# Yawning/secp256k1-voi

Measured on NVIDIA B200. Metric: ecdsa_verifies_per_sec, higher is better.
Workload: dtype u32 limbs (8x32, IMAD.WIDE.U32 carry chains)

## Files before the change

### secp256k1-voi_b200/csrc/api.cu

```cuda
#include "ctx.h"
#include "microbench.cuh"

__global__ void __launch_bounds__(S256_TPB) k_gen_table(apt *out, int wb, size_t total) {
    size_t idx = (size_t)blockIdx.x * blockDim.x + threadIdx.x;
    if (idx >= total) return;
    uint32_t w = (uint32_t)(idx >> wb), d = (uint32_t)(idx & ((1u << wb) - 1u));
    apt a;
    item_gen_multiple(a, w, d, wb);
    out[idx] = a;
}
__global__ void k_comb_bases(apt *bases) {
    uint32_t w = threadIdx.x;
    if (w < (uint32_t)COMB_NW) item_gen_multiple(bases[w], w, 1u, COMB_WB);
}
constexpr int COMB_RUN = 32;
static_assert(COMB_SZ % COMB_RUN == 0, "a run never straddles two windows");
__global__ void __launch_bounds__(S256_TPB) k_gen_comb(const apt *bases, size_t total, apt *out) {
    size_t e0 = ((size_t)blockIdx.x * blockDim.x + threadIdx.x) * COMB_RUN;
    if (e0 >= total) return;
    const apt B = bases[e0 / COMB_SZ];
    const uint32_t m = (uint32_t)(e0 % COMB_SZ) + 1u;
    pt buf[COMB_RUN];
    pt acc;
    pt_set_identity(acc);
// ... 16 lines not shown
    }
    fe_invert(inv, run);
#pragma unroll 1
    for (int i = COMB_RUN - 1; i >= 0; i--) {
        fe zi;
        apt a;
        fe_mul(zi, inv, pre[i]);
        fe_mul(inv, inv, buf[i].z);
        fe_mul(a.x, buf[i].x, zi);
        fe_mul(a.y, buf[i].y, zi);
        fe_normalize(a.x, a.x);
        fe_normalize(a.y, a.y);
        out[e0 + i] = a;
    }
}
template <int WB>
__global__ void __launch_bounds__(S256_TPB) k_gen_ct_table(apt *out) {
    constexpr int CT_SZ = ct_cfg<WB>::SZ, CT_NW = ct_cfg<WB>::NW, CT_WB = WB;
    uint32_t idx = blockIdx.x * blockDim.x + threadIdx.x;
    if (idx >= (uint32_t)(CT_NW * CT_SZ)) return;
    apt a;
    item_gen_multiple(a, idx / CT_SZ, idx % CT_SZ + 1u, CT_WB);
    out[idx] = a;
}

__global__ void __launch_bounds__(S256_TPB) k_decode_uncompressed(const uint8_t *pt65, size_t n, apt *aff,
                                                                  uint8_t *pvalid) {
    size_t i = (size_t)blockIdx.x * blockDim.x + threadIdx.x;
    if (i >= n) return;
    apt a;
    pvalid[i] = item_decode_uncompressed(a, pt65 + 65 * i);
    aff[i] = a;
}

__global__ void __launch_bounds__(S256_TPB) k_decode_compressed(const uint8_t *pt33, size_t n, apt *aff,
                                                                uint8_t *pvalid) {
    size_t i = (size_t)blockIdx.x * blockDim.x + threadIdx.x;
    if (i >= n) return;
    apt a;
    pvalid[i] = item_decode_compressed(a, pt33 + 33 * i);
    aff[i] = a;
}
__global__ void __launch_bounds__(S256_TPB) k_decode_sec1(const uint8_t *enc65, const uint8_t *len, size_t n, apt *aff,
                                                          uint8_t *pvalid) {
    size_t i = (size_t)blockIdx.x * blockDim.x + threadIdx.x;
    if (i >= n) return;
    const uint8_t *e = enc65 + 65 * i;
    apt a;
    a.x = fe_zero();
    a.y = fe_zero();
    uint8_t st = ST_INVALID;
    if (len[i] == 65)
        st = item_decode_uncompressed(a, e) ? ST_OK : ST_INVALID;
    else if (len[i] == 33)
        st = item_decode_compressed(a, e) ? ST_OK : ST_INVALID;
    else if (len[i] == 1 && e[0] == 0x00)
        st = ST_IDENTITY;
    pvalid[i] = st;
    aff[i] = a;
}
__global__ void __launch_bounds__(S256_TPB) k_encode_affine(const apt *aff, const uint8_t *pvalid, size_t n,
                                                            uint8_t *out65, uint8_t *status) {
    size_t i = (size_t)blockIdx.x * blockDim.x + threadIdx.x;
    if (i >= n) return;
    apt a = aff[i];
    uint32_t ok = pvalid[i] != 0;
    uint8_t *o = out65 + 65 * i;
    if (ok) {
        o[0] = 0x04;
        fe_to_be32(o + 1, a.x);
        fe_to_be32(o + 33, a.y);
    } else {
        for (int b = 0; b < 65; b++) o[b] = 0;
    }
    status[i] = ok ? ST_OK : ST_INVALID;
}
__global__ void __launch_bounds__(S256_TPB) k_encode_compressed(const apt *aff, const uint8_t *pvalid, size_t n,
                                                                uint8_t *out33, uint8_t *status) {
    size_t i = (size_t)blockIdx.x * blockDim.x + threadIdx.x;
    if (i >= n) return;
    apt a = aff[i];
    uint32_t ok = pvalid[i] != 0;
    uint8_t *o = out33 + 33 * i;
    if (ok) {
        o[0] = (uint8_t)(0x02u | fe_is_odd(a.y));
        fe_to_be32(o + 1, a.x);
    } else {
        for (int b = 0; b < 33; b++) o[b] = 0;
    }
    status[i] = ok ? ST_OK : ST_INVALID;
}
__global__ void __launch_bounds__(S256_TPB) k_encode_public_key(const apt *aff, const uint8_t *pvalid, size_t n,
                                                                uint8_t *out65, uint8_t *status) {
    size_t i = (size_t)blockIdx.x * blockDim.x + threadIdx.x;
    if (i >= n) return;
    apt a = aff[i];
    uint8_t *o = out65 + 65 * i;
    if (pvalid[i] == ST_OK) {
        o[0] = 0x04;
        fe_to_be32(o + 1, a.x);
        fe_to_be32(o + 33, a.y);
    } else {
        for (int b = 0; b < 65; b++) o[b] = 0;
    }
    status[i] = pvalid[i];
}

__global__ void __launch_bounds__(S256_TPB) k_decode_xonly(const uint8_t *pkx32, size_t n, apt *aff, uint8_t *pvalid) {
    size_t i = (size_t)blockIdx.x * blockDim.x + threadIdx.x;
    if (i >= n) return;
    apt a;
    pvalid[i] = item_decode_xonly(a, pkx32 + 32 * i);
    aff[i] = a;
}

__global__ void __launch_bounds__(S256_TPB) k_decode_recover(const uint8_t *sig65, size_t n, apt *aff,
                                                             uint8_t *pvalid) {
    size_t i = (size_t)blockIdx.x * blockDim.x + threadIdx.x;
    if (i >= n) return;
    apt a;
    pvalid[i] = item_decode_recover(a, sig65 + 65 * i);
    aff[i] = a;
}

template <int K, bool RECOVER>
__global__ void __launch_bounds__(S256_TPB, 4) k_ecdsa_scalars(const uint8_t *digest32, const uint8_t *sig, size_t n,
                                                            uint32_t flags, sc *u1, int8_t *dig1, int8_t *dig2,
                                                            uint8_t *sfl) {
    size_t stride = (n + K - 1) / K;
    size_t t = (size_t)blockIdx.x * blockDim.x + threadIdx.x;
    if (t >= stride) return;
    if (!RECOVER)
        group_ecdsa_scalars<K>(t, stride, n, digest32, sig, flags, u1, dig1, dig2, sfl);
    else
        group_recover_scalars<K>(t, stride, n, digest32, sig, u1, dig1, dig2, sfl);
}

__global__ void __launch_bounds__(S256_TPB) k_plain_scalars(const uint8_t *u1b, const uint8_t *u2b, size_t n, sc *u1,
                                                            int8_t *dig1, int8_t *dig2, uint8_t *sfl) {
    size_t i = (size_t)blockIdx.x * blockDim.x + threadIdx.x;
    if (i >= n) return;
    item_plain_scalars(i, n, u1b, u2b, u1, dig1, dig2, sfl);
}

__global__ void __launch_bounds__(S256_TPB) k_schnorr_scalars(const uint8_t *pkx32, const uint8_t *msg, size_t msg_len,
                                                              const uint8_t *sig64, size_t n, sc *u1, int8_t *dig1,
                                                              int8_t *dig2, uint8_t *sfl) {
    size_t i = (size_t)blockIdx.x * blockDim.x + threadIdx.x;
    if (i >= n) return;
    item_schnorr_scalars(i, n, pkx32, msg, msg_len, sig64, u1, dig1, dig2, sfl);
}

#ifndef S256_DSM_MINB
#define S256_DSM_MINB 4
#endif
#ifndef S256_DSM_TPB
#define S256_DSM_TPB S256_TPB
#endif
__device__ __forceinline__ void fe_shfl_xor(fe &r, const fe &a, int m) {
#pragma unroll
    for (int k = 0; k < 8; k++) r.v[k] = __shfl_xor_sync(0xFFFFFFFFu, a.v[k], m);
}
template <int TPB, class F>
__device__ __forceinline__ void cta_invert(F &f, fe &inv, const fe &c, fe *sh) {
    constexpr int PER = TPB / 32;
    sh[threadIdx.x] = c;
    __syncthreads();
    if (threadIdx.x < 32) {
        fe *mine = sh + threadIdx.x * PER;
        fe pre[PER];
        pre[0] = mine[0];
#pragma unroll
        for (int k = 1; k < PER; k++) f.mul(pre[k], pre[k - 1], mine[k]);
        fe all = pre[PER - 1], others, got;
        fe_shfl_xor(others, all, 1);
        f.mul(all, all, others);
#pragma unroll 1
        for (int m = 2; m < 32; m <<= 1) {
            fe_shfl_xor(got, all, m);
            f.mul(others, others, got);
            f.mul(all, all, got);
        }
        fe o;
        fe_invert(o, all);
        f.mul(o, o, others);
#pragma unroll
        for (int k = PER - 1; k >= 1; k--) {
            fe ck = mine[k], t;
            f.mul(t, o, pre[k - 1]);
            f.mul(o, o, ck);
            mine[k] = t;
        }
        mine[0] = o;
    }
    __syncthreads();
    inv = sh[threadIdx.x];
}
__global__ void __launch_bounds__(S256_DSM_TPB, S256_DSM_MINB)
    k_dsm(size_t n, const apt *aff, const sc *u1, const int8_t *dig1, const int8_t *dig2, const uint8_t *sfl, pt *tbl,
          pt *res, const apt *comb) {
    size_t i = (size_t)blockIdx.x * blockDim.x + threadIdx.x;
    if (i >= n) return;
    item_dsm(i, n, aff, u1, dig1, dig2, sfl, tbl, res, comb);
}

#ifndef S256_SM_MINB
#define S256_SM_MINB 4
#endif
__global__ void __launch_bounds__(S256_TPB, S256_SM_MINB)
    k_scalar_mult_ct(size_t n, const apt *aff, const uint8_t *k32, pt *tbl, pt *res) {
    size_t i = (size_t)blockIdx.x * blockDim.x + threadIdx.x;
#ifdef S256_CT_TABLE_GLOBAL
    if (i >= n) return;
    CtTableGlobal T{tbl + i * (size_t)DSM_TSTRIDE};
    item_scalar_mult_ct_affine(i, aff, k32, T, tbl + i * (size_t)DSM_TSTRIDE, res);
#else
    extern __shared__ uint4 ct_smem[];
    fe *sh = reinterpret_cast<fe *>(ct_smem);
    const bool live = i < n;
    fe_ops<true> f;
    fe zprod = fe_one(), inv;
    if (live) item_ctm_table(i, aff, tbl + i * (size_t)DSM_TSTRIDE, zprod);
    cta_invert<S256_TPB>(f, inv, zprod, sh);
    __syncthreads();
    if (!live) return;
    CtTableShared<S256_TPB> T{threadIdx.x, aff + i};
    item_ctm_ladder(i, aff, k32, T, tbl + i * (size_t)DSM_TSTRIDE, inv, res);
#endif
}
#ifdef S256_CT_TABLE_GLOBAL
constexpr size_t CT_SMEM_BYTES = 0;
#else
constexpr size_t CT_SMEM_BYTES = (size_t)(CTM_TS - 1) * 4 * S256_TPB * sizeof(uint4);
#endif
void s256_launch_scalar_mult_ct(size_t n, const apt *aff, const uint8_t *k32, pt *tbl, pt *res, cudaStream_t s) {
    if (n == 0) return;
    k_scalar_mult_ct<<<(unsigned)((n + S256_TPB - 1) / S256_TPB), S256_TPB, CT_SMEM_BYTES, s>>>(n, aff, k32, tbl, res);
}


__global__ void __launch_bounds__(S256_TPB) k_ecdsa_finish(size_t n, const pt *res, const uint8_t *sig64,
                                                           const uint8_t *pvalid, const uint8_t *sfl, uint8_t *ok) {
    size_t i = (size_t)blockIdx.x * blockDim.x + threadIdx.x;
    if (i >= n) return;
    pt R = res[i];
    uint32_t valid = (uint32_t)(pvalid[i] != 0) & (uint32_t)(sfl[i] & SFL_VALID);
    ok[i] = item_ecdsa_finish(R, sig64 + 64 * i, valid);
}

template <int K>
__global__ void __launch_bounds__(S256_TPB) k_finish_affine(size_t n, const pt *res, const uint8_t *pvalid,
                                                            const uint8_t *sfl, uint8_t *comb_status, int mode,
                                                            uint8_t *out, uint8_t *status, const uint8_t *sig64) {
    __shared__ uint4 stage[S256_TPB / 32][130];
    size_t stride = (((n + K - 1) / K) + 31) & ~(size_t)31;
    size_t t = (size_t)blockIdx.x * blockDim.x + threadIdx.x;
    if (t >= stride) return;
    group_finish<K>(t, stride, n, res, pvalid, sfl, comb_status, mode, out, status, sig64,
                    reinterpret_cast<uint8_t *>(stage[threadIdx.x / 32]));
}

__global__ void __launch_bounds__(S256_TPB) k_field_op(int op, const uint8_t *a32, const uint8_t *b32, size_t n,
                                                       uint8_t *out32) {
    size_t i = (size_t)blockIdx.x * blockDim.x + threadIdx.x;
    if (i >= n) return;
    if (op < 16 || op >= 20) {
        fe a, b, r;
        fe_from_be32(a, a32 + 32 * i);
        fe_from_be32(b, b32 + 32 * i);
        switch (op) {
            case 0: fe_mul(r, a, b); break;
            case 1: fe_add(r, a, b); break;
            case 2: fe_sub(r, a, b); break;
            case 3: fe_invert(r, a); break;
            case 4: fe_sqrt(r, a); break;
            case 5: fe_mul_small(r, a, 21u); break;
            case 6: fe_sqr(r, a); break;
            case 7: fe_invert_fermat(r, a); break;
            case 8: fe_mul_vt(r, a, b); break;
            case 9: fe_add_vt(r, a, b); break;
            case 10: fe_sub_vt(r, a, b); break;
            case 13: fe_mul_small_vt(r, a, 21u); break;
            case 14: fe_sqr_vt(r, a); break;
            case 15: fe_mul8_vt(r, a); break;
            case 20: fe_mul2_vt(r, a); break;
            case 21: fe_mul3_vt(r, a); break;
            case 22: fe_sub2_vt(r, a, b); break;
            case 23: fe_submul8_vt(r, a, b); break;
            case 24: fe_ops<false>::mul2add(r, a, b, b, a); break;
            case 25: fe_ops<false>::mul2sub(r, a, a, b, b); break;
            default: r = fe_zero();
        }
        fe_normalize(r, r);
        fe_to_be32(out32 + 32 * i, r);
    } else {
        sc a, b, r;
        sc_from_be32(a, a32 + 32 * i);
        sc_from_be32(b, b32 + 32 * i);
        switch (op) {
            case 16: sc_mul(r, a, b); break;
            case 17: sc_add(r, a, b); break;
            case 18: sc_invert(r, a); break;
            case 19: sc_invert_fermat(r, a); break;
            default: r = sc_zero();
        }
        sc_to_be32(out32 + 32 * i, r);
    }
}

extern "C" void *s256_host_alloc(size_t bytes) {
    void *p = nullptr;
    if (cudaHostAlloc(&p, bytes ? bytes : 1, cudaHostAllocPortable) != cudaSuccess) {
        cudaGetLastError();
        return nullptr;
    }
    return p;
}
extern "C" void s256_host_free(void *p) {
    if (p) cudaFreeHost(p);
}

extern "C" const char *s256_strerror(int code) {
    switch (code) {
        case S256_SUCCESS: return "success";
        case S256_ERR_NO_DEVICE: return "no usable CUDA device (sm_100 required; there is no CPU fallback)";
        case S256_ERR_CUDA: return "CUDA runtime error";
        case S256_ERR_ARG: return "invalid argument";
        case S256_ERR_NOMEM: return "out of memory";
        case S256_ERR_UNIMPLEMENTED: return "not implemented";
        case S256_ERR_NCCL: return "NCCL error";
        default: return "unknown error";
    }
}
extern "C" const char *s256_last_cuda_error(const s256_ctx *ctx) { return ctx ? ctx->last_err.c_str() : ""; }
extern "C" int s256_device(const s256_ctx *ctx) { return ctx ? ctx->device : -1; }
extern "C" uint64_t s256_launch_count(const s256_ctx *ctx) { return ctx ? ctx->launches.load() : 0; }

extern "C" void s256_free(s256_ctx *ctx) {
    if (!ctx) return;
    {
        dev_guard g(ctx->device);
        s256_internal_comm_release(ctx);
        void *ptrs[] = {ctx->comb, ctx->ct_tab, ctx->ct_tab_small, ctx->ct_tab_huge, ctx->aff, ctx->u1,   ctx->dig1, ctx->dig2, ctx->sfl, ctx->pvalid,
                        ctx->cstat, ctx->tbl,   ctx->res, ctx->in_a, ctx->in_b, ctx->in_c, ctx->out, ctx->st,
                        ctx->sink, ctx->msm_counts, ctx->msm_offsets, ctx->msm_cursor, ctx->msm_entries, ctx->msm_flag,
                        ctx->msm_buckets, ctx->msm_win, ctx->msm_acc, ctx->msm_tmp, ctx->msm_cub, ctx->msm_nsl, ctx->msm_sloff,
                        ctx->msm_perm, ctx->msm_hist, ctx->msm_range, ctx->msm_part, ctx->msm_sbkt, ctx->comm_buf, ctx->msm_aff2, ctx->msm_half, ctx->msm_bsum};
        for (void *p : ptrs)
            if (p) cudaFree(p);
        if (ctx->stream) cudaStreamDestroy(ctx->stream);
        if (ctx->stream2) cudaStreamDestroy(ctx->stream2);
        if (ctx->ev_decode) cudaEventDestroy(ctx->ev_decode);
        if (ctx->ev_idle) cudaEventDestroy(ctx->ev_idle);
        for (cudaEvent_t e : ctx->ev_pipe)
// ... 880 lines not shown
```

### secp256k1-voi_b200/csrc/jac.cuh

```cuda
#pragma once
#include "point.cuh"

namespace s256 {

template <class F>
S256_HD void jac_double(F &fo, pt &v, const pt &p) {
    fe a, b, c, d, e, f, t, z3;
    fo.sqr(a, p.x);
    fo.sqr(b, p.y);
    fo.sqr(c, b);
#ifndef S256_JDBL_3M4S
    fo.add(t, p.x, b);
    fo.sqr(t, t);
    fo.sub(t, t, a);
    fo.sub(t, t, c);
    fo.mul2(d, t);
#else
    fo.mul(t, p.x, b);
    fo.mul2(t, t);
    fo.mul2(d, t);
#endif
    fo.mul3(e, a);
    fo.sqr(f, e);
    fo.mul(z3, p.y, p.z);
    fo.mul2(v.z, z3);
    fo.sub2(t, f, d);
    v.x = t;
    fo.sub(t, d, t);
    fo.mul(f, e, t);
    fo.submul8(v.y, f, c);
}
template <class F>
S256_HD void jac_add_mixed_nocheck(F &fo, pt &v, const pt &p, const fe &x2, const fe &y2) {
    fe zz, u2, s2, h, r, hh, hhh, w, t, x3;
    fo.sqr(zz, p.z);
    fo.mul(u2, x2, zz);
    fo.mul(s2, y2, p.z);
    fo.mul(s2, s2, zz);
    fo.sub(h, u2, p.x);
    fo.sub(r, s2, p.y);
    fo.sqr(hh, h);
    fo.mul(hhh, h, hh);
    fo.mul(w, p.x, hh);
    fo.mul(v.z, p.z, h);
    fo.sqr(x3, r);
    fo.sub(x3, x3, hhh);
    fo.sub2(x3, x3, w);
    fo.sub(t, w, x3);
    fo.mul2sub(v.y, r, t, p.y, hhh);
    v.x = x3;
}

template <class F>
S256_HD void jac_dblu(F &fo, fe &x2, fe &y2, fe &x1, fe &y1, const fe &x, const fe &y) {
    fe a, b, c, d, e, t;
    fo.sqr(a, x);
    fo.sqr(b, y);
    fo.sqr(c, b);
    fo.add(t, x, b);
    fo.sqr(t, t);
    fo.sub(t, t, a);
    fo.sub(t, t, c);
    fo.mul2(d, t);
    fo.mul3(e, a);
    fo.sqr(t, e);
    fo.sub2(x2, t, d);
    fo.sub(t, d, x2);
    fo.mul(a, e, t);
    fo.submul8(y2, a, c);
    x1 = d;
    fo.mul8(y1, c);
}
template <class F>
S256_HD void jac_zaddu(F &fo, fe &x1, fe &y1, fe &x2, fe &y2, fe &u) {
    fe c, w1, w2, r, t;
    fo.sub(u, x1, x2);
    fo.sqr(c, u);
    fo.mul(w1, x1, c);
    fo.mul(w2, x2, c);
    fo.sub(r, y1, y2);
    fo.sub(t, w1, w2);
    fo.mul(y1, y1, t);
    fo.sqr(t, r);
    fo.sub(t, t, w1);
    fo.sub(x2, t, w2);
    fo.sub(t, w1, x2);
    fo.mul(c, r, t);
    fo.sub(y2, c, y1);
    x1 = w1;
}

template <class F>
S256_HD void jac_add_mixed_var(F &fo, pt &acc, uint32_t &inf, const fe &x2, const fe &y2) {
    if (inf) {
        acc.x = x2;
        acc.y = y2;
        acc.z = fe_one();
        inf = 0u;
        return;
    }
    fe zz, u2, s2, h, r, hh, hhh, w, t, x3;
    fo.sqr(zz, acc.z);
    fo.mul(u2, x2, zz);
    fo.mul(s2, y2, acc.z);
    fo.mul(s2, s2, zz);
    fo.sub(h, u2, acc.x);
    fo.sub(r, s2, acc.y);
    if (fe_is_zero(h)) {
        if (!fe_is_zero(r)) {
            inf = 1u;
            acc.x = acc.y = acc.z = fe_zero();
        } else {
            jac_double(fo, acc, acc);
        }
        return;
    }
    fo.sqr(hh, h);
    fo.mul(hhh, h, hh);
    fo.mul(w, acc.x, hh);
    fo.mul(acc.z, acc.z, h);
    fo.sqr(x3, r);
    fo.sub(x3, x3, hhh);
    fo.sub2(x3, x3, w);
    fo.sub(t, w, x3);
    fo.mul2sub(acc.y, r, t, acc.y, hhh);
    acc.x = x3;
}

template <class F>
S256_HD void jac_to_projective(F &fo, pt &v, const pt &p, uint32_t inf) {
    if (inf) {
        pt_set_identity(v);
        return;
    }
    fe zz;
    fo.sqr(zz, p.z);
    fo.mul(v.x, p.x, p.z);
    v.y = p.y;
    fo.mul(v.z, zz, p.z);
}

}
```

### secp256k1-voi_b200/csrc/kernels.cuh

```cuda
#pragma once
#include "fe.cuh"
#include "point.cuh"
#include "jac.cuh"
#include "sc.cuh"
#include "sha256.cuh"

namespace s256 {

#ifndef S256_W
#define S256_W 5
#endif
constexpr int DSM_W = S256_W;
constexpr int DSM_ND = glv_recode<DSM_W>::ND;
constexpr int DSM_TS = 1 << (DSM_W - 1);
#ifndef S256_DSM_RCB
#define S256_DSM_JAC 1
static_assert(DSM_TS >= 4, "the co-Z table needs at least two chain steps (item_dsm_table)");
constexpr int DSM_TSTRIDE = (64 * DSM_TS + 32 * (DSM_TS - 2) + 95) / 96;
#else
constexpr int DSM_TSTRIDE = DSM_TS;
#endif
#ifndef S256_COMB_WB
#define S256_COMB_WB 22
#endif
// ... 114 lines not shown
    sfl[i] = (uint8_t)((valid ? SFL_VALID : 0) | (neg1 ? SFL_NEG1 : 0) | (neg2 ? SFL_NEG2 : 0));
}

struct ecdsa_parsed {
    sc r, s, e;
    uint32_t valid;
};
S256_HD void item_ecdsa_parse(ecdsa_parsed &o, const uint8_t *digest32, const uint8_t *sig64, uint32_t flags) {
    uint32_t rr = sc_from_be32(o.r, sig64);
    uint32_t sr = sc_from_be32(o.s, sig64 + 32);
    uint32_t ok = (1u - rr) & (1u - sr) & (1u - sc_is_zero(o.r)) & (1u - sc_is_zero(o.s));
    if (flags & FLAG_REJECT_MALLEABLE) ok &= 1u - sc_is_gt_half_n(o.s);
    sc_from_be32(o.e, digest32);
    sc one = sc_one();
    sc_cmov(o.s, one, o.s, ok);
    o.valid = ok;
}

template <int K>
S256_HD void group_ecdsa_scalars(size_t t, size_t stride, size_t n, const uint8_t *digest32, const uint8_t *sig64,
                                 uint32_t flags, sc *u1_out, int8_t *dig1, int8_t *dig2, uint8_t *sfl) {
    sc pre[K];
    sc run = sc_one();
    ecdsa_parsed p;
    for (int m = 0; m < K; m++) {
        size_t i = t + (size_t)m * stride;
        pre[m] = run;
        if (i < n) {
            item_ecdsa_parse(p, digest32 + 32 * i, sig64 + 64 * i, flags);
            sc_mul(run, run, p.s);
        }
    }
    sc inv;
    sc_invert(inv, run);
    for (int m = K - 1; m >= 0; m--) {
        size_t i = t + (size_t)m * stride;
        if (i >= n) continue;
        item_ecdsa_parse(p, digest32 + 32 * i, sig64 + 64 * i, flags);
        sc sinv, u1, u2;
        sc_mul(sinv, inv, pre[m]);
        sc_mul(inv, inv, p.s);
        sc_mul(u1, p.e, sinv);
        sc_mul(u2, p.r, sinv);
        item_store_scalars(u1, u2, p.valid, i, n, u1_out, dig1, dig2, sfl);
    }
}

S256_HD void item_plain_scalars(size_t i, size_t n, const uint8_t *u1b, const uint8_t *u2b, sc *u1_out, int8_t *dig1,
                                int8_t *dig2, uint8_t *sfl) {
    sc u1, u2;
    sc_from_be32(u1, u1b + 32 * i);
    sc_from_be32(u2, u2b + 32 * i);
    item_store_scalars(u1, u2, 1u, i, n, u1_out, dig1, dig2, sfl);
}

S256_HD uint8_t item_decode_xonly(apt &out, const uint8_t *pkx32) {
    fe x;
    fe_from_be32(x, pkx32);
    return item_decompress(out, x, fe_limbs_are_canonical(x), 0u);
}
S256_HD uint8_t item_decode_recover(apt &out, const uint8_t *sig65) {
    uint32_t v = sig65[64];
    sc r;
    uint32_t ok = 1u - sc_from_be32(r, sig65);
    ok &= (uint32_t)(v < 4);
    fe x;
#pragma unroll
    for (int k = 0; k < 8; k++) x.v[k] = r.v[k];
    if (v & 2u) {
        fe nn = fe_group_order();
        uint64_t acc = 0;
#pragma unroll
        for (int k = 0; k < 8; k++) {
            acc = (acc >> 32) + x.v[k] + nn.v[k];
            x.v[k] = (uint32_t)acc;
        }
        ok &= (1u - (uint32_t)(acc >> 32)) & fe_limbs_are_canonical(x);
    }
    return item_decompress(out, x, ok, v & 1u);
}

template <int K>
S256_HD void group_recover_scalars(size_t t, size_t stride, size_t n, const uint8_t *digest32, const uint8_t *sig65,
                                   sc *u1_out, int8_t *dig1, int8_t *dig2, uint8_t *sfl) {
    sc pre[K];
    sc run = sc_one();
    const sc one = sc_one();
    ecdsa_parsed p;
    for (int m = 0; m < K; m++) {
        size_t i = t + (size_t)m * stride;
        pre[m] = run;
        if (i < n) {
            item_ecdsa_parse(p, digest32 + 32 * i, sig65 + 65 * i, 0u);
            sc_cmov(p.r, one, p.r, p.valid);
            sc_mul(run, run, p.r);
        }
    }
    sc inv;
    sc_invert(inv, run);
    for (int m = K - 1; m >= 0; m--) {
        size_t i = t + (size_t)m * stride;
        if (i >= n) continue;
        item_ecdsa_parse(p, digest32 + 32 * i, sig65 + 65 * i, 0u);
        sc_cmov(p.r, one, p.r, p.valid);
        sc rinv, ne, a, b2;
        sc_mul(rinv, inv, pre[m]);
        sc_mul(inv, inv, p.r);
        sc_neg(ne, p.e);
        sc_mul(a, ne, rinv);
        sc_mul(b2, p.s, rinv);
        item_store_scalars(a, b2, p.valid, i, n, u1_out, dig1, dig2, sfl);
    }
}

S256_HD void item_schnorr_scalars(size_t i, size_t n, const uint8_t *pkx32, const uint8_t *msg, size_t msg_len,
                                  const uint8_t *sig64, sc *u1_out, int8_t *dig1, int8_t *dig2, uint8_t *sfl) {
    const uint8_t *sg = sig64 + 64 * i;
    fe r;
    fe_from_be32(r, sg);
    sc s, e, ne;
    uint32_t ok = fe_limbs_are_canonical(r) & (1u - sc_from_be32(s, sg + 32));
    uint8_t eb[32];
    if (msg_len == 32) {
        uint32_t rw[8], pw[8], mw[8], ew[8];
        be32_words(rw, sg);
        be32_words(pw, pkx32 + 32 * i);
        be32_words(mw, msg + 32 * i);
        bip340_tagged_96(ew, TAG_CHALLENGE, rw, pw, mw);
        words_be32(eb, ew);
    } else {
        bip340_challenge(eb, sg, pkx32 + 32 * i, msg + msg_len * i, msg_len);
    }
    sc_from_be32(e, eb);
    sc_neg(ne, e);
    item_store_scalars(s, ne, ok, i, n, u1_out, dig1, dig2, sfl);
}

S256_HD void pt_fetch64(pt &r, const pt *p) {
#if defined(__CUDA_ARCH__) && !defined(S256_DSM_LD32)
    const uint2 *q = reinterpret_cast<const uint2 *>(p);
#pragma unroll
    for (int k = 0; k < 4; k++) {
        uint2 a = q[k], b = q[4 + k], c = q[8 + k];
        r.x.v[2 * k] = a.x; r.x.v[2 * k + 1] = a.y;
        r.y.v[2 * k] = b.x; r.y.v[2 * k + 1] = b.y;
        r.z.v[2 * k] = c.x; r.z.v[2 * k + 1] = c.y;
    }
#else
    r = *p;
#endif
}
constexpr bool DSM_VT = true;
#if defined(S256_DSM_JAC)
S256_HD void apt_fetch64(apt &r, const apt *p) {
#if defined(__CUDA_ARCH__) && !defined(S256_DSM_LD32)
    const uint2 *q = reinterpret_cast<const uint2 *>(p);
#pragma unroll
    for (int k = 0; k < 4; k++) {
        uint2 a = q[k], b = q[4 + k];
        r.x.v[2 * k] = a.x; r.x.v[2 * k + 1] = a.y;
        r.y.v[2 * k] = b.x; r.y.v[2 * k + 1] = b.y;
    }
#else
    r = *p;
#endif
}
constexpr int DSM_U_OFF = 64 * DSM_TS;
template <class F>
S256_HD void item_dsm_table(F &f, size_t i, const apt *aff, pt *tbl) {
    char *base = reinterpret_cast<char *>(tbl + i * (size_t)DSM_TSTRIDE);
    apt *A = reinterpret_cast<apt *>(base);
    fe *U = reinterpret_cast<fe *>(base + DSM_U_OFF);
    apt P = aff[i];
    apt p, q;
    jac_dblu(f, q.x, q.y, p.x, p.y, P.x, P.y);
    A[1] = q;
#if defined(__CUDA_ARCH__)
#pragma unroll 1
#endif
    for (int k = 2; k < DSM_TS; k++) {
        fe u;
        jac_zaddu(f, p.x, p.y, q.x, q.y, u);
        A[k] = q;
        U[k - 2] = u;
    }
    A[0] = p;
    fe r = U[DSM_TS - 3];
#if defined(__CUDA_ARCH__)
#pragma unroll 1
#endif
    for (int k = DSM_TS - 1; k >= 2; k--) {
        if (k < DSM_TS - 1) {
            fe uk = U[k - 2];
            f.mul(r, r, uk);
        }
        apt a = A[k - 1];
        fe rr;
        f.sqr(rr, r);
        f.mul(a.x, a.x, rr);
        f.mul(rr, rr, r);
        f.mul(a.y, a.y, rr);
        A[k - 1] = a;
    }
    fe zall;
    f.mul2(zall, P.y);
    f.mul(zall, zall, r);
    U[0] = zall;
}
template <class F>
S256_HD void item_dsm_ladder(F &f, size_t i, size_t n, const sc *u1s, const int8_t *dig1, const int8_t *dig2,
                             const uint8_t *sfl, pt *tbl, pt *res, const apt *comb) {
    char *base = reinterpret_cast<char *>(tbl + i * (size_t)DSM_TSTRIDE);
    const apt *A = reinterpret_cast<const apt *>(base);
    uint32_t fl = sfl[i];
    pt acc;
    acc.x = fe_zero();
    acc.y = fe_zero();
    acc.z = fe_zero();
    uint32_t inf = 1u;
    const fe beta = fe_beta();
#if defined(__CUDA_ARCH__)
#pragma unroll 1
#endif
    for (int s = DSM_ND - 1; s >= 0; s--) {
        int da = dig1[(size_t)s * n + i];
        int db = dig2[(size_t)s * n + i];
#if defined(__CUDA_ARCH__) && !defined(S256_DSM_NO_PREFETCH)
        {
            int ma = da < 0 ? -da : da, mb = db < 0 ? -db : db;
            if (ma) asm volatile("prefetch.global.L1 [%0];" ::"l"(A + (ma - 1)));
            if (mb) asm volatile("prefetch.global.L1 [%0];" ::"l"(A + (mb - 1)));
        }
#endif
        if (s != DSM_ND - 1) {
#if defined(__CUDA_ARCH__)
#pragma unroll 1
#endif
            for (int k = 0; k < DSM_W; k++) jac_double(f, acc, acc);
        }
#if defined(__CUDA_ARCH__)
#pragma unroll 1
#endif
        for (int h = 0; h < 2; h++) {
            int d = h ? db : da;
            if (d != 0) {
                uint32_t neg = (uint32_t)(d < 0) ^ ((fl >> (1 + h)) & 1u);
                int mag = d < 0 ? -d : d;
                apt q;
                apt_fetch64(q, A + (mag - 1));
                if (h) f.mul(q.x, q.x, beta);
                if (neg) {
                    fe z = fe_zero();
                    f.sub(q.y, z, q.y);
                }
                jac_add_mixed_var(f, acc, inf, q.x, q.y);
            }
        }
    }
    if (!inf) {
        fe zall = reinterpret_cast<const fe *>(base + DSM_U_OFF)[0];
        f.mul(acc.z, acc.z, zall);
    }
    sc u1 = u1s[i];
    uint32_t carry = 0;
#if defined(__CUDA_ARCH__)
#pragma unroll 1
#endif
    for (int w = 0; w < COMB_NW; w++) {
        int32_t d = comb_digit(u1, w, carry);
        if (d != 0) {
            uint32_t mag = (uint32_t)(d < 0 ? -d : d);
            apt g = comb[(size_t)w * COMB_SZ + (mag - 1u)];
            if (d < 0) {
                fe z = fe_zero();
                f.sub(g.y, z, g.y);
            }
            jac_add_mixed_var(f, acc, inf, g.x, g.y);
        }
    }
    pt out;
    jac_to_projective(f, out, acc, inf);
    res[i] = out;
}
S256_HD void item_dsm(size_t i, size_t n, const apt *aff, const sc *u1s, const int8_t *dig1, const int8_t *dig2,
                      const uint8_t *sfl, pt *tbl, pt *res, const apt *comb) {
    fe_ops<DSM_VT> f;
    item_dsm_table(f, i, aff, tbl);
    item_dsm_ladder(f, i, n, u1s, dig1, dig2, sfl, tbl, res, comb);
}
#else
S256_HD void item_dsm(size_t i, size_t n, const apt *aff, const sc *u1s, const int8_t *dig1, const int8_t *dig2,
                      const uint8_t *sfl, pt *tbl, pt *res, const apt *comb) {
    pt *T = tbl + i * (size_t)DSM_TS;
    {
        apt P = aff[i];
        pt cur;
        pt_from_affine(cur, P);
        T[0] = cur;
#if defined(__CUDA_ARCH__)
#pragma unroll 1
#endif
        for (int k = 2; k <= DSM_TS; k += 2) {
            pt h = T[k / 2 - 1];
            pt_double<DSM_VT>(cur, h);
            T[k - 1] = cur;
            if (k < DSM_TS) {
                pt_add_mixed<DSM_VT>(cur, cur, P.x, P.y);
                T[k] = cur;
            }
        }
    }
    uint32_t fl = sfl[i];
    pt acc;
    pt_set_identity(acc);
    const fe beta = fe_beta();
#if defined(__CUDA_ARCH__)
#pragma unroll 1
#endif
    for (int s = DSM_ND - 1; s >= 0; s--) {
        int da = dig1[(size_t)s * n + i];
        int db = dig2[(size_t)s * n + i];
#if defined(__CUDA_ARCH__) && !defined(S256_DSM_NO_PREFETCH)
        {
            int ma = da < 0 ? -da : da, mb = db < 0 ? -db : db;
            if (ma) {
                const char *r = reinterpret_cast<const char *>(T + (ma - 1));
                asm volatile("prefetch.global.L1 [%0];" ::"l"(r));
                asm volatile("prefetch.global.L1 [%0];" ::"l"(r + 64));
            }
            if (mb) {
                const char *r = reinterpret_cast<const char *>(T + (mb - 1));
                asm volatile("prefetch.global.L1 [%0];" ::"l"(r));
                asm volatile("prefetch.global.L1 [%0];" ::"l"(r + 64));
            }
        }
#endif
        if (s != DSM_ND - 1) {
#if defined(__CUDA_ARCH__)
#pragma unroll 1
#endif
            for (int k = 0; k < DSM_W; k++) pt_double<DSM_VT>(acc, acc);
        }
#if defined(__CUDA_ARCH__)
#pragma unroll 1
#endif
        for (int h = 0; h < 2; h++) {
            int d = h ? db : da;
            if (d != 0) {
                uint32_t neg = (uint32_t)(d < 0) ^ ((fl >> (1 + h)) & 1u);
                int mag = d < 0 ? -d : d;
                pt q;
                pt_fetch64(q, T + (mag - 1));
                if (h) fe_ops<DSM_VT>::mul(q.x, q.x, beta);
                if (neg) {
                    fe z = fe_zero();
                    fe_ops<DSM_VT>::sub(q.y, z, q.y);
                }
                if (s == DSM_ND - 1 && h == 0)
                    acc = q;
                else
                    pt_add<DSM_VT>(acc, acc, q);
            }
        }
    }
    sc u1 = u1s[i];
    uint32_t carry = 0;
#if defined(__CUDA_ARCH__)
#pragma unroll 1
#endif
    for (int w = 0; w < COMB_NW; w++) {
        int32_t d = comb_digit(u1, w, carry);
        if (d != 0) {
            uint32_t mag = (uint32_t)(d < 0 ? -d : d);
            apt g = comb[(size_t)w * COMB_SZ + (mag - 1u)];
            if (d < 0) {
                fe z = fe_zero();
                fe_ops<DSM_VT>::sub(g.y, z, g.y);
            }
            pt_add_mixed<DSM_VT>(acc, acc, g.x, g.y);
        }
    }
    res[i] = acc;
}

#endif

S256_HD uint8_t item_ecdsa_finish(const pt &R, const uint8_t *sig64, uint32_t valid) {
    fe r, rn, t;
    fe_from_be32(r, sig64);
    uint32_t ok = valid & (1u - pt_is_identity(R));
    fe_mul(t, r, R.z);
    uint32_t m1 = fe_equal(t, R.x);
    fe nn = fe_group_order();
    uint64_t acc = 0;
#pragma unroll
    for (int k = 0; k < 8; k++) {
        acc = (acc >> 32) + r.v[k] + nn.v[k];
        rn.v[k] = (uint32_t)acc;
    }
    uint32_t fits = (1u - (uint32_t)(acc >> 32)) & fe_limbs_are_canonical(rn);
    fe_mul(t, rn, R.z);
    uint32_t m2 = fits & fe_equal(t, R.x);
    return (uint8_t)(ok & (m1 | m2));
}

S256_HD void pt_fetch(pt &r, const pt *p) {
#if defined(__CUDA_ARCH__)
    const uint4 *q = reinterpret_cast<const uint4 *>(p);
    uint4 a0 = q[0], a1 = q[1], a2 = q[2], a3 = q[3], a4 = q[4], a5 = q[5];
    r.x.v[0] = a0.x; r.x.v[1] = a0.y; r.x.v[2] = a0.z; r.x.v[3] = a0.w;
    r.x.v[4] = a1.x; r.x.v[5] = a1.y; r.x.v[6] = a1.z; r.x.v[7] = a1.w;
    r.y.v[0] = a2.x; r.y.v[1] = a2.y; r.y.v[2] = a2.z; r.y.v[3] = a2.w;
    r.y.v[4] = a3.x; r.y.v[5] = a3.y; r.y.v[6] = a3.z; r.y.v[7] = a3.w;
    r.z.v[0] = a4.x; r.z.v[1] = a4.y; r.z.v[2] = a4.z; r.z.v[3] = a4.w;
    r.z.v[4] = a5.x; r.z.v[5] = a5.y; r.z.v[6] = a5.z; r.z.v[7] = a5.w;
#else
    r = *p;
#endif
}
S256_HD void fe_fetch(fe &r, const fe *p) {
#if defined(__CUDA_ARCH__)
    const uint4 *q = reinterpret_cast<const uint4 *>(p);
    uint4 a0 = q[0], a1 = q[1];
    r.v[0] = a0.x; r.v[1] = a0.y; r.v[2] = a0.z; r.v[3] = a0.w;
    r.v[4] = a1.x; r.v[5] = a1.y; r.v[6] = a1.z; r.v[7] = a1.w;
#else
    r = *p;
#endif
}

template <int K>
// ... 595 lines not shown
```

Measured before the change: 58.24 million.

## Reduce register pressure in DSM ladder by deferring table loads and hoisting doubling

Restructures the mixed-add so the table point's x/y are loaded lazily through a row functor, right before use, and beta-multiplication and negation happen inside it. The rare doubling case inside the add is deferred to a single shared doubling call in the outer loop instead of being inlined in every add site. The patch also narrows the thread index to 32 bits, reorders a few field ops in doubling, and raises min blocks per SM from 4 to 5. Together these aim to cut live registers and code size so more warps fit per SM, at the risk of spills under the tighter launch bound and a more complex control flow.

```diff
diff --git a/secp256k1-voi_b200/csrc/api.cu b/secp256k1-voi_b200/csrc/api.cu
--- a/secp256k1-voi_b200/csrc/api.cu
+++ b/secp256k1-voi_b200/csrc/api.cu
@@ -192,7 +192,7 @@
 }
 
 #ifndef S256_DSM_MINB
-#define S256_DSM_MINB 4
+#define S256_DSM_MINB 5
 #endif
 #ifndef S256_DSM_TPB
 #define S256_DSM_TPB S256_TPB
@@ -239,7 +239,7 @@
 __global__ void __launch_bounds__(S256_DSM_TPB, S256_DSM_MINB)
     k_dsm(size_t n, const apt *aff, const sc *u1, const int8_t *dig1, const int8_t *dig2, const uint8_t *sfl, pt *tbl,
           pt *res, const apt *comb) {
-    size_t i = (size_t)blockIdx.x * blockDim.x + threadIdx.x;
+    uint32_t i = blockIdx.x * blockDim.x + threadIdx.x;
     if (i >= n) return;
     item_dsm(i, n, aff, u1, dig1, dig2, sfl, tbl, res, comb);
 }
diff --git a/secp256k1-voi_b200/csrc/jac.cuh b/secp256k1-voi_b200/csrc/jac.cuh
--- a/secp256k1-voi_b200/csrc/jac.cuh
+++ b/secp256k1-voi_b200/csrc/jac.cuh
@@ -6,23 +6,24 @@
 template <class F>
 S256_HD void jac_double(F &fo, pt &v, const pt &p) {
     fe a, b, c, d, e, f, t, z3;
+    fo.sqr(b, p.y);
+    fo.mul(z3, p.y, p.z);
     fo.sqr(a, p.x);
-    fo.sqr(b, p.y);
-    fo.sqr(c, b);
 #ifndef S256_JDBL_3M4S
     fo.add(t, p.x, b);
+    fo.sqr(c, b);
     fo.sqr(t, t);
     fo.sub(t, t, a);
     fo.sub(t, t, c);
     fo.mul2(d, t);
 #else
     fo.mul(t, p.x, b);
+    fo.sqr(c, b);
     fo.mul2(t, t);
     fo.mul2(d, t);
 #endif
     fo.mul3(e, a);
     fo.sqr(f, e);
-    fo.mul(z3, p.y, p.z);
     fo.mul2(v.z, z3);
     fo.sub2(t, f, d);
     v.x = t;
@@ -90,18 +91,20 @@
     x1 = w1;
 }
 
-template <class F>
-S256_HD void jac_add_mixed_var(F &fo, pt &acc, uint32_t &inf, const fe &x2, const fe &y2) {
+template <class F, class Row>
+S256_HD void jac_add_mixed_row(F &fo, pt &acc, uint32_t &inf, const Row &row) {
     if (inf) {
-        acc.x = x2;
-        acc.y = y2;
+        row.x(fo, acc.x);
+        row.y(fo, acc.y);
         acc.z = fe_one();
         inf = 0u;
         return;
     }
-    fe zz, u2, s2, h, r, hh, hhh, w, t, x3;
+    fe zz, x2, y2, u2, s2, h, r, hh, hhh, w, t, x3;
     fo.sqr(zz, acc.z);
+    row.x(fo, x2);
     fo.mul(u2, x2, zz);
+    row.y(fo, y2);
     fo.mul(s2, y2, acc.z);
     fo.mul(s2, s2, zz);
     fo.sub(h, u2, acc.x);
@@ -111,20 +114,33 @@
             inf = 1u;
             acc.x = acc.y = acc.z = fe_zero();
         } else {
-            jac_double(fo, acc, acc);
+            row.dbl(fo, acc);
         }
         return;
     }
     fo.sqr(hh, h);
+    fo.mul(acc.z, acc.z, h);
     fo.mul(hhh, h, hh);
     fo.mul(w, acc.x, hh);
-    fo.mul(acc.z, acc.z, h);
     fo.sqr(x3, r);
     fo.sub(x3, x3, hhh);
     fo.sub2(x3, x3, w);
     fo.sub(t, w, x3);
     fo.mul2sub(acc.y, r, t, acc.y, hhh);
     acc.x = x3;
+}
+struct jac_affine_row {
+    const fe &x2, &y2;
+    template <class F>
+    S256_HD void x(F &, fe &r) const { r = x2; }
+    template <class F>
+    S256_HD void y(F &, fe &r) const { r = y2; }
+    template <class F>
+    S256_HD void dbl(F &fo, pt &acc) const { jac_double(fo, acc, acc); }
+};
+template <class F>
+S256_HD void jac_add_mixed_var(F &fo, pt &acc, uint32_t &inf, const fe &x2, const fe &y2) {
+    jac_add_mixed_row(fo, acc, inf, jac_affine_row{x2, y2});
 }
 
 template <class F>
diff --git a/secp256k1-voi_b200/csrc/kernels.cuh b/secp256k1-voi_b200/csrc/kernels.cuh
--- a/secp256k1-voi_b200/csrc/kernels.cuh
+++ b/secp256k1-voi_b200/csrc/kernels.cuh
@@ -290,19 +290,38 @@
 }
 constexpr bool DSM_VT = true;
 #if defined(S256_DSM_JAC)
-S256_HD void apt_fetch64(apt &r, const apt *p) {
+S256_HD void fe_fetch64(fe &r, const fe *p) {
 #if defined(__CUDA_ARCH__) && !defined(S256_DSM_LD32)
     const uint2 *q = reinterpret_cast<const uint2 *>(p);
 #pragma unroll
     for (int k = 0; k < 4; k++) {
-        uint2 a = q[k], b = q[4 + k];
-        r.x.v[2 * k] = a.x; r.x.v[2 * k + 1] = a.y;
-        r.y.v[2 * k] = b.x; r.y.v[2 * k + 1] = b.y;
+        uint2 a = q[k];
+        r.v[2 * k] = a.x; r.v[2 * k + 1] = a.y;
     }
 #else
     r = *p;
 #endif
 }
+struct dsm_row {
+    const apt *p;
+    uint32_t lam, neg;
+    uint32_t *owed;
+    template <class F>
+    S256_HD void dbl(F &, pt &) const { *owed = 1u; }
+    template <class F>
+    S256_HD void x(F &f, fe &r) const {
+        fe_fetch64(r, &p->x);
+        if (lam) f.mul(r, r, fe_beta());
+    }
+    template <class F>
+    S256_HD void y(F &f, fe &r) const {
+        fe_fetch64(r, &p->y);
+        if (neg) {
+            fe z = fe_zero();
+            f.sub(r, z, r);
+        }
+    }
+};
 constexpr int DSM_U_OFF = 64 * DSM_TS;
 template <class F>
 S256_HD void item_dsm_table(F &f, size_t i, const apt *aff, pt *tbl) {
@@ -317,10 +336,8 @@
 #pragma unroll 1
 #endif
     for (int k = 2; k < DSM_TS; k++) {
-        fe u;
-        jac_zaddu(f, p.x, p.y, q.x, q.y, u);
+        jac_zaddu(f, p.x, p.y, q.x, q.y, U[k - 2]);
         A[k] = q;
-        U[k - 2] = u;
     }
     A[0] = p;
     fe r = U[DSM_TS - 3];
@@ -340,8 +357,8 @@
         f.mul(a.y, a.y, rr);
         A[k - 1] = a;
     }
-    fe zall;
-    f.mul2(zall, P.y);
+    fe zall, y = aff[i].y;
+    f.mul2(zall, y);
     f.mul(zall, zall, r);
     U[0] = zall;
 }
@@ -356,7 +373,6 @@
     acc.y = fe_zero();
     acc.z = fe_zero();
     uint32_t inf = 1u;
-    const fe beta = fe_beta();
 #if defined(__CUDA_ARCH__)
 #pragma unroll 1
 #endif
@@ -370,51 +386,50 @@
             if (mb) asm volatile("prefetch.global.L1 [%0];" ::"l"(A + (mb - 1)));
         }
 #endif
-        if (s != DSM_ND - 1) {
-#if defined(__CUDA_ARCH__)
-#pragma unroll 1
-#endif
-            for (int k = 0; k < DSM_W; k++) jac_double(f, acc, acc);
-        }
-#if defined(__CUDA_ARCH__)
-#pragma unroll 1
-#endif
-        for (int h = 0; h < 2; h++) {
-            int d = h ? db : da;
-            if (d != 0) {
-                uint32_t neg = (uint32_t)(d < 0) ^ ((fl >> (1 + h)) & 1u);
-                int mag = d < 0 ? -d : d;
-                apt q;
-                apt_fetch64(q, A + (mag - 1));
-                if (h) f.mul(q.x, q.x, beta);
-                if (neg) {
-                    fe z = fe_zero();
-                    f.sub(q.y, z, q.y);
+        int nd = s != DSM_ND - 1 ? DSM_W : 0, h = 0;
+        for (;;) {
+#if defined(__CUDA_ARCH__)
+#pragma unroll 1
+#endif
+            for (int k = 0; k < nd; k++) jac_double(f, acc, acc);
+            uint32_t owed = 0u;
+#if defined(__CUDA_ARCH__)
+#pragma unroll 1
+#endif
+            for (; h < 2 && !owed; h++) {
+                int d = h ? db : da;
+                if (d != 0) {
+                    uint32_t neg = (uint32_t)(d < 0) ^ ((fl >> (1 + h)) & 1u);
+                    int mag = d < 0 ? -d : d;
+                    jac_add_mixed_row(f, acc, inf, dsm_row{A + (mag - 1), (uint32_t)h, neg, &owed});
                 }
-                jac_add_mixed_var(f, acc, inf, q.x, q.y);
-            }
+            }
+            if (!owed) break;
+            nd = 1;
         }
     }
     if (!inf) {
         fe zall = reinterpret_cast<const fe *>(base + DSM_U_OFF)[0];
         f.mul(acc.z, acc.z, zall);
     }
-    sc u1 = u1s[i];
+    const sc &u1 = u1s[i];
     uint32_t carry = 0;
 #if defined(__CUDA_ARCH__)
 #pragma unroll 1
 #endif
-    for (int w = 0; w < COMB_NW; w++) {
-        int32_t d = comb_digit(u1, w, carry);
-        if (d != 0) {
-            uint32_t mag = (uint32_t)(d < 0 ? -d : d);
-            apt g = comb[(size_t)w * COMB_SZ + (mag - 1u)];
-            if (d < 0) {
-                fe z = fe_zero();
-                f.sub(g.y, z, g.y);
-            }
-            jac_add_mixed_var(f, acc, inf, g.x, g.y);
-        }
+    for (int w = 0; w < COMB_NW;) {
+        uint32_t owed = 0u;
+#if defined(__CUDA_ARCH__)
+#pragma unroll 1
+#endif
+        for (; w < COMB_NW && !owed; w++) {
+            int32_t d = comb_digit(u1, w, carry);
+            if (d != 0) {
+                uint32_t mag = (uint32_t)(d < 0 ? -d : d);
+                jac_add_mixed_row(f, acc, inf, dsm_row{comb + ((size_t)w * COMB_SZ + (mag - 1u)), 0u, (uint32_t)(d < 0), &owed});
+            }
+        }
+        if (owed) jac_double(f, acc, acc);
     }
     pt out;
     jac_to_projective(f, out, acc, inf);
```

New measurement: 59.82 million, median of 6. 2.7% higher.
